# GuildOfWeavers/distaff

Measured on AMD Instinct MI355X. Metric: trace_cells_per_sec, higher is better.
Workload: dtype u128 (prime field 2^128-45*2^40+1, 4x u32 limbs)

## Files before the change

distaff_amd/csrc/air_kernel.h:

```cpp
#pragma once
#include "ctx.h"
#include <type_traits>

#ifndef AIR_THREADS
#define AIR_THREADS 128
#endif
#ifdef AIR_CONVOY
#define AIR_SYNC() __builtin_amdgcn_s_barrier()
#else
#define AIR_SYNC()
#endif
#ifndef AIR_WAVES_PER_SIMD
#define AIR_WAVES_PER_SIMD 2
#endif
constexpr int air_waves_per_simd(int sd, int slcap, int sect) {
    (void)sd; (void)slcap; (void)sect;
#ifdef AIR_WAVES_FORCE
    return AIR_WAVES_FORCE;
#else
    return AIR_WAVES_PER_SIMD;
#endif
}

struct AirConsts { fe sponge_mds[16], sponge_inv_mds[16], hasher_mds[36], hasher_inv_mds[36]; };

struct AirArgs {
    const fe* lde;
    fe* out;
    const fe* coef;
    const fe* tc;
    const fe* periodic;
    const AirConsts* consts;
    fe* partial;
    fe* ev[10];
    const fe* tw_lo; const fe* tw_hi; uint32_t lo_bits;
    unsigned long long* bad_step;
    size_t n, col_stride;
    uint32_t log_n, log_N, log_b, W, ctx_depth, loop_depth, stack_depth;
    uint32_t cl, ll, sl;
    uint32_t coset_step;
    uint32_t q0;
    uint32_t num_inputs, num_outputs;
    fe inputs[8], outputs[8], program_hash[2], op_count;
};



__device__ __forceinline__ fe dpow(const AirArgs& a, uint64_t e) {
    uint32_t l = (uint32_t)e & ((1u << a.lo_bits) - 1u), h = (uint32_t)(e >> a.lo_bits);
    fe v = a.tw_lo[l];
    return h ? fe_mul(v, a.tw_hi[h]) : v;
}

__device__ __forceinline__ fe bnot(const fe& v) { return fe_sub(fe_one(), v); }
__device__ __forceinline__ fe is_bin(const fe& v) { return fe_sub(fe_sqr(v), v); }

template <int Wd>
__device__ __forceinline__ void matmul(fe* s, const fe* m) {
    fe r[Wd];
#pragma unroll
    for (int i = 0; i < Wd; i++) {
        fe_acc A; fe_acc_zero(A);
#pragma unroll
        for (int j = 0; j < Wd; j++) fe_acc_mac(A, m[i * Wd + j], s[j]);
        r[i] = fe_acc_reduce(A);
    }
#pragma unroll
    for (int i = 0; i < Wd; i++) s[i] = r[i];
}

template <int I, int N, class F>
__device__ __forceinline__ void static_for_air(F&& f) {
    if constexpr (I < N) { f(std::integral_constant<int, I>{}); static_for_air<I + 1, N>(f); }
}

struct StackRows { fe o[12], nw[8], hd0; int sl; };
#define ST_AUX0 8
#define ST_AUX1 9

template <int OP, int I> constexpr bool st_has() {
    constexpr bool slot = I < 8, aux0 = I == ST_AUX0, aux1 = I == ST_AUX1;
    switch (OP) {
        case 0x00: case 0x01: case 0x05: case 0x06: case 0x07: return slot || aux0;
        case 0x02: case 0x0E: return slot || aux0;
        case 0x03: case 0x04: case 0x08: case 0x09: case 0x0C: case 0x0D: return slot;
        case 0x0A: case 0x0B: return slot || aux0 || aux1;
        case 0x10: return I >= 1 && slot;
        case 0x11: return I >= 2 && slot;
        case 0x12: case 0x13: case 0x14: case 0x15: return slot;
        case 0x18: return slot && I != 1;
        case 0x19: case 0x1A: case 0x1B: case 0x1C: case 0x1D: return slot;
        default: return false;
    }
}

template <int OP, int I>
__device__ __forceinline__ fe st_term(const StackRows& s) {
    const fe* o = s.o; const fe* nw = s.nw;
    constexpr int i = I < 8 ? I : 0;
    auto L = [&](int num) {
        if (i + num < 8) return fe_sub(o[i + num < 8 ? i + num : 0], nw[i]);
        return i + num < s.sl ? fe_sub(o[i + num < 12 ? i + num : 0], nw[i]) : nw[i];
    };
    auto R = [&](int num) { return fe_sub(o[i - num < 0 ? 0 : i - num], nw[i]); };
    auto C = [&]() { return fe_sub(o[i], nw[i]); };
    auto sel = [&](const fe& c, const fe& x, const fe& y) { return fe_add(y, fe_mul(c, fe_sub(x, y))); };
    if constexpr (OP == 0x00) { if constexpr (I == ST_AUX0) return bnot(o[0]); else return L(1); }
    else if constexpr (OP == 0x01) { if constexpr (I == ST_AUX0) return fe_sub(o[0], o[1]); else return L(2); }
    else if constexpr (OP == 0x02) {
        const fe diff = fe_sub(o[1], o[2]);
        if constexpr (I == ST_AUX0) return fe_mul(nw[0], diff);
        else if constexpr (I == 0) return fe_sub(nw[0], bnot(fe_mul(diff, o[0])));
        else return L(2);
    }
    else if constexpr (OP == 0x03) return L(1);
    else if constexpr (OP == 0x04) return L(4);
    else if constexpr (OP == 0x05) {
        if constexpr (I == ST_AUX0) return is_bin(o[2]);
        else if constexpr (I == 0) return fe_sub(nw[0], sel(o[2], o[0], o[1]));
        else return L(2);
    }
    else if constexpr (OP == 0x06) {
// ... 81 lines not shown
    auto rdiff = [&](int j) { return (SDK != 0 && j >= SDK) ? StDesc{3, 0} : StDesc{2, j}; };
    auto L = [&](int num) { return i + num < 8 ? diff(i + num) : (DEEP ? StDesc{5, -1} : StDesc{3, 0}); };
    auto R = [&](int num) { return diff(i - num < 0 ? 0 : i - num); };
    switch (op) {
        case 0x00: return L(1);
        case 0x01: return L(2);
        case 0x02: return i == 0 ? StDesc{5, -1} : L(2);
        case 0x03: return L(1);
        case 0x04: return L(4);
        case 0x05: return i == 0 ? StDesc{5, -1} : L(2);
        case 0x06: return i < 2 ? (o4_zero ? rdiff(i + 2) : StDesc{5, -1}) : L(4);
        case 0x07: return i < 4 ? (o4_zero ? rdiff(i) : StDesc{5, -1}) : L(2);
        case 0x08: case 0x0B: return i == 0 ? StDesc{5, -1} : L(1);
        case 0x09: case 0x0A: return i == 0 ? StDesc{5, 102} : L(1);
        case 0x0C: case 0x0D: case 0x0E: return i == 0 ? StDesc{5, -1} : diff(i);
        case 0x10: return R(1);
        case 0x11: return R(2);
        case 0x12: return i == 0 ? rdiff(0) : R(1);
        case 0x13: return i < 2 ? rdiff(i) : R(2);
        case 0x14: return i < 4 ? rdiff(i) : R(4);
        case 0x15: return i < 2 ? StDesc{3, 0} : R(2);
        case 0x18: return i == 0 ? StDesc{5, -1} : diff(i);
        case 0x19: return i < 4 ? rdiff(i ^ 2) : diff(i);
        case 0x1A: return rdiff(i ^ 4);
        case 0x1B: return i < 4 ? rdiff((i + 3) & 3) : diff(i);
        case 0x1C: return rdiff((i + 7) & 7);
        case 0x1D: return i == 1 ? StDesc{3, 0} : (i < 4 ? StDesc{5, -1} : diff(i));
        default: return StDesc{0, 0};
    }
}
struct StMerge { int n; int kind[4], j[4], lead[4]; int sgn[4][4]; };
template <int BASE, int I, int SDK, bool DEEP>
constexpr StMerge st_merge() {
    StMerge m{};
    for (int a = 0; a < 4; a++) {
        const StDesc d = st_desc<SDK, DEEP>(BASE + a, I);
        bool has = false;
        switch (a) { case 0: has = st_has<BASE, I>(); break; case 1: has = st_has<BASE + 1, I>(); break; case 2: has = st_has<BASE + 2, I>(); break; default: has = st_has<BASE + 3, I>(); }
        if (!has || d.kind == 0) continue;
        const int cls = d.kind == 5 ? 5 : (d.kind <= 2 ? 1 : 3);
        const int sign = (d.kind == 2 || d.kind == 4) ? -1 : 1;
        int e = -1;
        for (int k = 0; k < m.n; k++) {
            const int kc = m.kind[k] == 5 ? 5 : (m.kind[k] <= 2 ? 1 : 3);
            if (kc != cls) continue;
            if (cls == 3 || (cls == 1 && m.j[k] == d.j) || (cls == 5 && d.j >= 100 && m.j[k] == d.j)) e = k;
        }
        if (e < 0) { e = m.n++; m.kind[e] = d.kind; m.j[e] = d.j; m.lead[e] = a; m.sgn[e][a] = 1; }
        else { const int lead_sign = (m.kind[e] == 2 || m.kind[e] == 4) ? -1 : 1; m.sgn[e][a] = sign * lead_sign; }
    }
    return m;
}

struct StackHigh { fe push, cmp, rescr, keep; fe resc[6]; };

template <int I, uint32_t GROUPS>
__device__ __forceinline__ void st_high_degree(fe_acc& outer, const StackRows& s, const StackHigh& h) {
    if constexpr (I < 8) {
        const fe* o = s.o; const fe* nw = s.nw;
        if constexpr (I >= 1 && (GROUPS & AG_PUSH) != 0) fe_acc_mac(outer, h.push, fe_sub(o[I - 1 < 0 ? 0 : I - 1], nw[I]));
        if constexpr ((GROUPS & AG_CMP) != 0) {
            const fe x_bit = nw[1], y_bit = nw[2], not_set = nw[3];
            fe v;
            if constexpr (I == 0) v = is_bin(x_bit);
            else if constexpr (I == 1) v = is_bin(y_bit);
            else if constexpr (I == 2) v = fe_sub(nw[4], fe_add(o[4], fe_mul(fe_mul(x_bit, bnot(y_bit)), not_set)));
            else if constexpr (I == 3) v = fe_sub(nw[5], fe_add(o[5], fe_mul(fe_mul(y_bit, bnot(x_bit)), not_set)));
            else if constexpr (I == 4) v = fe_sub(nw[6], fe_add(o[6], fe_mul(y_bit, o[0])));
            else if constexpr (I == 5) v = fe_sub(nw[7], fe_add(o[7], fe_mul(x_bit, o[0])));
            else if constexpr (I == 6) v = fe_sub(not_set, fe_mul(bnot(o[5]), bnot(o[4])));
            else v = fe_sub(fe_double(nw[0]), o[0]);
            fe_acc_mac(outer, h.cmp, v);
        }
        if constexpr ((GROUPS & (AG_RESCR | AG_KEEP)) != 0) {
            const fe keep = fe_sub(o[I < 8 ? I : 0], nw[I < 8 ? I : 0]);
            if constexpr ((GROUPS & AG_RESCR) != 0) { if constexpr (I < 6) fe_acc_mac(outer, h.rescr, h.resc[I < 6 ? I : 0]); else fe_acc_mac(outer, h.rescr, keep); }
            if constexpr ((GROUPS & AG_KEEP) != 0) fe_acc_mac(outer, h.keep, keep);
        }
    }
}

template <int I, uint32_t GROUPS> constexpr bool st_touches() {
    if (I >= 8) return (GROUPS & AG_LOW0) != 0;
    return (GROUPS & (AG_LOW0 | AG_LOW1 | AG_HIGH)) != 0;
}

template <int I, uint32_t GROUPS, int SDK, bool DEEP>
__device__ __forceinline__ fe st_output(const StackRows& s, const fe* lo2, const fe& lo0h, const fe* mid, const fe* top, const StackHigh& h) {
    fe_acc outer; fe_acc_zero(outer);
    static_for_air<0, 2>([&](auto c_) {
        constexpr int c = decltype(c_)::value;
        if constexpr (((GROUPS >> (4 * c)) & 0xFu) != 0) {
            fe_acc middle; fe_acc_zero(middle);
            static_for_air<0, 4>([&](auto b_) {
                constexpr int b = decltype(b_)::value;
                constexpr int base = 4 * b + 16 * c;
                if constexpr ((GROUPS & AG_LOW(c, b)) != 0) {
                    static constexpr StMerge M = st_merge<base, I, SDK, DEEP>();
                    if constexpr (M.n > 0) {
                        fe_acc inner; fe_acc_zero(inner);
                        static_for_air<0, M.n>([&](auto e_) {
                            constexpr int e = decltype(e_)::value;
                            fe cf = (base == 0 && M.lead[e] == 0) ? lo0h : lo2[M.lead[e]];
                            static_for_air<0, 4>([&](auto a_) {
                                constexpr int a = decltype(a_)::value;
                                if constexpr (a != M.lead[e] && M.sgn[e][a] != 0) {
                                    const fe other = (base == 0 && a == 0) ? lo0h : lo2[a];
                                    cf = M.sgn[e][a] > 0 ? fe_add(cf, other) : fe_sub(cf, other);
                                }
                            });
                            constexpr int ii = I < 8 ? I : 0;
                            fe term;
                            if constexpr (M.kind[e] == 1) term = fe_sub(s.o[M.j[e]], s.nw[ii]);
                            else if constexpr (M.kind[e] == 2) term = fe_sub(s.nw[ii], s.o[M.j[e]]);
                            else if constexpr (M.kind[e] == 3) term = s.nw[ii];
                            else if constexpr (M.kind[e] == 4) term = fe_neg(s.nw[ii]);
                            else term = st_term<base + M.lead[e], I>(s);
                            fe_acc_mac(inner, cf, term);
                        });
                        fe_acc_mac(middle, mid[b], fe_acc_reduce(inner));
                    }
                }
            });
            fe_acc_mac(outer, top[c], fe_acc_reduce(middle));
        }
    });
    if constexpr ((GROUPS & AG_HIGH) != 0) st_high_degree<I, GROUPS>(outer, s, h);
    return fe_acc_reduce(outer);
}

template <uint32_t ACC_MASK>
struct Acc {
    fe_acc res_acc;
    fe_acc adj_acc[6];
    fe res, adj[6];
    bool nonzero;
    const fe* tc; uint32_t nc;
    __device__ __forceinline__ void emit(uint32_t cidx, int slot, const fe& d) {
        nonzero |= !fe_is_zero(d);
        fe_acc_mac(res_acc, d, tc[cidx]);
        if ((ACC_MASK >> slot) & 1u) fe_acc_mac(adj_acc[slot], d, tc[nc + cidx]);
        else adj[slot] = fe_add(adj[slot], fe_mul(d, tc[nc + cidx]));
    }
};

template <int CL, int LL, int SD, int SLCAP, int SECT, uint32_t GROUPS, int FLAGS>
__global__ void __launch_bounds__(AIR_THREADS, air_waves_per_simd(SD, SLCAP, SECT)) air_kernel(AirArgs a) {
    constexpr bool FIRST = (FLAGS & AF_FIRST) != 0, LAST = (FLAGS & AF_LAST) != 0, EV_IN = (FLAGS & AF_EV_IN) != 0, EV_OUT = (FLAGS & AF_EV_OUT) != 0;
    constexpr int SL = SD ? (SD > 8 ? SD : 8) : SLCAP;
    constexpr bool DEEP = SD == 0 && SLCAP == 12;
    const int cl = (int)a.cl, ll = (int)a.ll;
    const int sl = SD ? SL : (int)a.sl;
    const int sd = SD ? SD : (int)a.stack_depth;
    const fe* c_sponge_mds = a.consts->sponge_mds; const fe* c_sponge_inv_mds = a.consts->sponge_inv_mds;
    const fe* c_hasher_mds = a.consts->hasher_mds; const fe* c_hasher_inv_mds = a.consts->hasher_inv_mds;
    const size_t k = (size_t)blockIdx.x * AIR_THREADS + threadIdx.x;
    if (k >= a.n) return;
    const uint32_t ql = blockIdx.y;
    const uint32_t qg = a.q0 + ql;
    const uint32_t jl = ql * a.coset_step;
    const size_t kn = (k + 1 == a.n) ? 0 : k + 1;
    const fe* cur_p = a.lde + (size_t)jl * a.n + k;
    const fe* nxt_p = a.lde + (size_t)jl * a.n + kn;
    const size_t cs = a.col_stride;
#define CUR(c) cur_p[(size_t)(c) * cs]
#define NXT(c) nxt_p[(size_t)(c) * cs]

    const uint64_t nmask = ((uint64_t)1 << a.log_N) - 1;
    const uint64_t gi = ((uint64_t)k << a.log_b) + (uint64_t)qg * a.coset_step;
    const uint32_t step = (uint32_t)(((uint64_t)k << 3) + qg);
    const uint64_t n64 = a.n;

    const fe c_opc = CUR(0), n_opc = NXT(0);
    fe c_sp[4], n_sp[4], cf[3], ld[5], hd[2], n_cf[3];
#pragma unroll
    for (int i = 0; i < 4; i++) { c_sp[i] = CUR(1 + i); n_sp[i] = NXT(1 + i); }
#pragma unroll
    for (int i = 0; i < 3; i++) { cf[i] = CUR(5 + i); n_cf[i] = NXT(5 + i); }
#pragma unroll
    for (int i = 0; i < 5; i++) ld[i] = CUR(8 + i);
#pragma unroll
    for (int i = 0; i < 2; i++) hd[i] = CUR(13 + i);
    fe c_ctx[CL], n_ctx[CL], c_lp[LL], n_lp[LL], o[SL], nw[SL];
    {
        uint32_t col = 15;
#pragma unroll
        for (int i = 0; i < CL; i++) { bool on = (uint32_t)i < a.ctx_depth; c_ctx[i] = on ? CUR(col + i) : fe_zero(); n_ctx[i] = on ? NXT(col + i) : fe_zero(); }
        col += a.ctx_depth;
#pragma unroll
        for (int i = 0; i < LL; i++) { bool on = (uint32_t)i < a.loop_depth; c_lp[i] = on ? CUR(col + i) : fe_zero(); n_lp[i] = on ? NXT(col + i) : fe_zero(); }
        col += a.loop_depth;
#pragma unroll
        for (int i = 0; i < SL; i++) { bool on = i < sd; o[i] = on ? CUR(col + i) : fe_zero(); nw[i] = on ? NXT(col + i) : fe_zero(); }
    }

    if constexpr ((SECT & 1) != 0) {
        const fe xp = dpow(a, (gi * (6 * n64 + 2)) & nmask);
        const fe one = fe_one();
#pragma unroll 1
        for (int pass = 0; pass < 2; pass++) {
            const fe* cc = a.coef + pass * 94;
            fe_acc R, A; fe_acc_zero(R); fe_acc_zero(A);
            auto term = [&](const fe& v, uint32_t idx) { fe_acc_mac(R, v, cc[idx]); fe_acc_mac(A, v, cc[idx + 1]); };
            term(pass ? fe_sub(c_opc, a.op_count) : c_opc, 0);
            if (pass == 0) { for (int i = 0; i < 4; i++) term(c_sp[i], 2 + 2 * i); }
            else { for (int i = 0; i < 2; i++) term(fe_sub(c_sp[i], a.program_hash[i]), 2 + 2 * i); }
            for (int i = 0; i < 3; i++) term(pass ? fe_sub(cf[i], one) : cf[i], 10 + 2 * i);
            for (int i = 0; i < 5; i++) term(pass ? fe_sub(ld[i], one) : ld[i], 16 + 2 * i);
            for (int i = 0; i < 2; i++) term(pass ? fe_sub(hd[i], one) : hd[i], 26 + 2 * i);
            for (int i = 0; i < CL; i++) if (i < cl) term(c_ctx[i], 30 + 2 * i);
            for (int i = 0; i < LL; i++) if (i < ll) term(c_lp[i], 62 + 2 * i);
            const uint32_t nio = pass ? a.num_outputs : a.num_inputs;
// ... 121 lines not shown
                fe_acc_mac(A, ccpy, fe_sub(c_ctx[i], n_ctx[i]));
                const fe v = fe_acc_reduce(A);
                acc.emit(20 + i, 2, v);
            }
#pragma unroll
            for (int i = 0; i < LL; i++) {
                if (i >= ll) break;
                fe v = fe_mul(lcpy, fe_sub(c_lp[i], n_lp[i]));
                if (i >= 1) v = fe_add(v, fe_mul(f_loop, fe_sub(c_lp[i - 1 < 0 ? 0 : i - 1], n_lp[i])));
                v = fe_add(v, fe_mul(f_break, i + 1 < ll ? fe_sub(c_lp[i + 1 < LL ? i + 1 : 0], n_lp[i]) : n_lp[i]));
                acc.emit(20 + cl + i, 2, v);
            }
        } else {
            auto ctx_cur = [&](int i) { return (uint32_t)i < a.ctx_depth ? CUR(15 + i) : fe_zero(); };
            auto ctx_nxt = [&](int i) { return (uint32_t)i < a.ctx_depth ? NXT(15 + i) : fe_zero(); };
            const uint32_t lcol = 15 + a.ctx_depth;
            auto lp_cur = [&](int i) { return (uint32_t)i < a.loop_depth ? CUR(lcol + i) : fe_zero(); };
            auto lp_nxt = [&](int i) { return (uint32_t)i < a.loop_depth ? NXT(lcol + i) : fe_zero(); };
#pragma unroll 1
            for (int i = 0; i < cl; i++) {
                const fe ni = ctx_nxt(i);
                fe_acc A; fe_acc_zero(A);
                fe_acc_mac(A, push, fe_sub(i == 0 ? c_sp[0] : ctx_cur(i - 1), ni));
                fe_acc_mac(A, pop, i + 1 < cl ? fe_sub(ctx_cur(i + 1), ni) : ni);
                fe_acc_mac(A, ccpy, fe_sub(ctx_cur(i), ni));
                acc.emit(20 + i, 2, fe_acc_reduce(A));
            }
#pragma unroll 1
            for (int i = 0; i < ll; i++) {
                const fe ni = lp_nxt(i);
                fe_acc A; fe_acc_zero(A);
                fe_acc_mac(A, lcpy, fe_sub(lp_cur(i), ni));
                if (i >= 1) fe_acc_mac(A, f_loop, fe_sub(lp_cur(i - 1), ni));
                fe_acc_mac(A, f_break, i + 1 < ll ? fe_sub(lp_cur(i + 1), ni) : ni);
                acc.emit(20 + cl + i, 2, fe_acc_reduce(A));
            }
        }
    }

    constexpr bool NESTED = SD == 4 || (SD == 0 && SLCAP == 8) || DEEP;
    static_assert(NESTED ? (SECT & 120) == 0 : GROUPS == 0, "nested-sum instances select stack operations with GROUPS, the per-operation instance with SECT");
    if constexpr (NESTED && (GROUPS & AG_STACK_ALL & ~AG_DEEP) != 0) {
        constexpr int NS = SD == 4 ? 4 : 8;
        StackRows rows;
#pragma unroll
        for (int i = 0; i < 8; i++) { rows.o[i] = o[i]; rows.nw[i] = nw[i]; }
#pragma unroll
        for (int i = 8; i < 12; i++) rows.o[i] = DEEP ? o[i < SL ? i : 0] : fe_zero();
        rows.hd0 = hd[0];
        rows.sl = DEEP ? sl : 8;
        const fe lo0h = fe_mul(lo2[0], hd[0]);
        StackHigh high;
        high.push = hdf[0]; high.cmp = hdf[1]; high.rescr = hdf[2]; high.keep = fe_add(begin_flag, noop_flag);
        if constexpr ((GROUPS & AG_RESCR) != 0) {
            constexpr int NZ = (SD != 0 && SD < 6) ? SD : 6;
            fe os[6], ns[6];
#pragma unroll
            for (int i = 0; i < 6; i++) os[i] = i < NZ ? fe_cube(fe_add(o[i], per[8 + i])) : per[23 + i];
            matmul<6>(os, c_hasher_mds);
            constexpr int NR = NS < 6 ? NS : 6;
#pragma unroll
            for (int i = 0; i < NR; i++) {
                fe_acc A; fe_acc_zero(A);
#pragma unroll
                for (int j = 0; j < NZ; j++) fe_acc_mac(A, c_hasher_inv_mds[i * 6 + j], nw[j]);
                ns[i] = fe_acc_reduce(A);
            }
#pragma unroll
            for (int i = 0; i < NR; i++) high.resc[i] = fe_sub(fe_sub(fe_cube(ns[i]), per[14 + i]), os[i]);
        }
        AIR_SYNC();
        const uint32_t sbase = 20 + cl + ll;
        static_for_air<0, NS + 2>([&](auto k_) {
            constexpr int kk = decltype(k_)::value;
            constexpr int I = kk < NS ? kk : (kk == NS ? ST_AUX0 : ST_AUX1);
            constexpr bool touched = st_touches<I, GROUPS>();
            if constexpr (touched || !EV_OUT) {
                if (I >= 8 || I < sd) {
                    fe v = fe_zero();
                    if constexpr (touched) v = st_output<I, GROUPS, SD, DEEP>(rows, lo2, lo0h, mid, top, high);
                    fe* slot = a.ev[I] + pidx;
                    if constexpr (EV_IN) v = touched ? fe_add(v, *slot) : *slot;
                    if constexpr (EV_OUT) *slot = v;
                    else acc.emit(I >= 8 ? sbase + (I - 8) : sbase + 2 + I, 4, v);
                }
            } else if constexpr (!EV_IN) {
                a.ev[I][pidx] = fe_zero();
            }
            AIR_SYNC();
        });
    }
    if constexpr (!NESTED && (SECT & 120) != 0) {
        constexpr int SLR = SL;
        fe ev[SLR], aux0 = fe_zero(), aux1 = fe_zero();
#pragma unroll
        for (int i = 0; i < SLR; i++) ev[i] = fe_zero();
        auto agg = [&](int i, const fe& f, const fe& v) { if (i < sd) ev[i] = fe_add(ev[i], fe_mul(f, v)); };
        auto copy_from = [&](int from, const fe& f) {
#pragma unroll
            for (int i = 0; i < SLR; i++) if (i >= from && i < sl) agg(i, f, fe_sub(o[i], nw[i]));
        };
        auto rshift = [&](int num, const fe& f) {
#pragma unroll
            for (int i = 0; i < SLR; i++) if (i >= num && i < sl) agg(i, f, fe_sub(o[i - num < 0 ? 0 : i - num], nw[i]));
        };
        auto lshift = [&](int from, int num, const fe& f) {
#pragma unroll
            for (int i = 0; i < SLR; i++) {
                if (i >= from - num && i < sl - num) agg(i, f, fe_sub(o[i + num < SL ? i + num : 0], nw[i]));
                else if (i >= sl - num && i < sl) agg(i, f, nw[i]);
            }
        };
        fe f;
        constexpr bool HD_FUSED = false;
        if constexpr (!NESTED && (SECT & 8) != 0) {
        f = LDF(0x12); agg(0, f, fe_sub(nw[0], o[0]));
        rshift(1, fe_add(LDF(0x10), f));
        f = LDF(0x13); agg(0, f, fe_sub(nw[0], o[0])); agg(1, f, fe_sub(nw[1], o[1]));
        f = LDF(0x15); agg(0, f, nw[0]); agg(1, f, nw[1]);
        rshift(2, fe_add(fe_add(LDF(0x11), LDF(0x13)), LDF(0x15)));
        f = LDF(0x14);
#pragma unroll
        for (int i = 0; i < 4; i++) agg(i, f, fe_sub(nw[i], o[i]));
        rshift(4, f);
        lshift(1, 1, fe_add(assert_flag, LDF(0x03)));
        aux0 = fe_add(aux0, fe_mul(assert_flag, fe_sub(fe_one(), o[0])));
        lshift(2, 2, LDF(0x01));
        aux0 = fe_add(aux0, fe_mul(LDF(0x01), fe_sub(o[0], o[1])));
        lshift(4, 4, LDF(0x04));
        f = LDF(0x18); agg(0, f, fe_sub(nw[0], o[1])); agg(0, f, fe_sub(nw[1], o[0])); copy_from(2, f);
        f = LDF(0x19); agg(0, f, fe_sub(nw[0], o[2])); agg(1, f, fe_sub(nw[1], o[3])); agg(2, f, fe_sub(nw[2], o[0])); agg(3, f, fe_sub(nw[3], o[1])); copy_from(4, f);
        f = LDF(0x1A);
#pragma unroll
// ... 66 lines not shown
            f = hdf[1];
            fe x_bit = nw[1], y_bit = nw[2], not_set = nw[3];
            agg(0, f, is_bin(x_bit)); agg(1, f, is_bin(y_bit));
            fe bit_gt = fe_mul(x_bit, bnot(y_bit)), bit_lt = fe_mul(y_bit, bnot(x_bit));
            agg(2, f, fe_sub(nw[4], fe_add(o[4], fe_mul(bit_gt, not_set))));
            agg(3, f, fe_sub(nw[5], fe_add(o[5], fe_mul(bit_lt, not_set))));
            agg(4, f, fe_sub(nw[6], fe_add(o[6], fe_mul(y_bit, o[0]))));
            agg(5, f, fe_sub(nw[7], fe_add(o[7], fe_mul(x_bit, o[0]))));
            agg(6, f, fe_sub(not_set, fe_mul(bnot(o[5]), bnot(o[4]))));
            agg(7, f, fe_sub(fe_double(nw[0]), o[0]));
            copy_from(8, f);
        }
        copy_from(0, fe_add(begin_flag, noop_flag));
        }
        if constexpr (!HD_FUSED && (SECT & 64) != 0) {
        {
            f = hdf[2];
            fe os[6], ns[6];
#pragma unroll
            for (int i = 0; i < 6; i++) os[i] = fe_cube(fe_add(o[i], per[8 + i]));
            matmul<6>(os, c_hasher_mds);
#pragma unroll
            for (int i = 0; i < 6; i++) ns[i] = nw[i];
            matmul<6>(ns, c_hasher_inv_mds);
#pragma unroll
            for (int i = 0; i < 6; i++) ns[i] = fe_sub(fe_cube(ns[i]), per[14 + i]);
#pragma unroll
            for (int i = 0; i < 6; i++) agg(i, f, fe_sub(ns[i], os[i]));
            copy_from(6, f);
        }
        }

        const uint32_t sbase = 20 + cl + ll;
        if constexpr ((SECT & 40) != 0) { acc.emit(sbase, 4, aux0); acc.emit(sbase + 1, 4, aux1); }
#pragma unroll
        for (int i = 0; i < SLR; i++) if (i < sd) acc.emit(sbase + 2 + i, 4, ev[i]);
    }
    if constexpr (DEEP && (GROUPS & AG_DEEP) != 0) {
        {
            const uint32_t sbase = 20 + cl + ll;
            const fe lo_all = fe_add(fe_add(lo2[0], lo2[1]), fe_add(lo2[2], lo2[3]));
            fe fl1, fl2, fl4, fr1, fr2, fr4, fcp;
            { fe_acc A; fe_acc_zero(A); fe_acc_mac(A, mid[0], lo2[3]); fe_acc_mac(A, mid[2], lo_all); fl1 = fe_add(fe_mul(top[0], fe_acc_reduce(A)), assert_flag); }
            { fe_acc A; fe_acc_zero(A); fe_acc_mac(A, mid[0], fe_add(lo2[1], lo2[2])); fe_acc_mac(A, mid[1], fe_add(lo2[1], lo2[3])); fl2 = fe_mul(top[0], fe_acc_reduce(A)); }
            fl4 = fe_mul(top[0], fe_mul(mid[1], fe_add(lo2[0], lo2[2])));
            fr1 = fe_add(fe_mul(top[1], fe_mul(mid[0], fe_add(lo2[0], lo2[2]))), hdf[0]);
            { fe_acc A; fe_acc_zero(A); fe_acc_mac(A, mid[0], fe_add(lo2[1], lo2[3])); fe_acc_mac(A, mid[1], lo2[1]); fr2 = fe_mul(top[1], fe_acc_reduce(A)); }
            fr4 = fe_mul(top[1], fe_mul(mid[1], lo2[0]));
            {
                fe_acc A; fe_acc_zero(A); fe_acc_mac(A, mid[2], lo_all); fe_acc_mac(A, mid[3], fe_add(lo2[0], lo2[1]));
                fe_acc B; fe_acc_zero(B); fe_acc_mac(B, top[1], fe_acc_reduce(A)); fe_acc_mac(B, top[0], fe_mul(mid[3], fe_add(fe_add(lo2[0], lo2[1]), lo2[2])));
                fcp = fe_add(fe_add(fe_acc_reduce(B), fe_add(hdf[1], hdf[2])), fe_add(begin_flag, noop_flag));
            }
            const uint32_t scol = 15 + a.ctx_depth + a.loop_depth;
#pragma unroll 1
            for (int i = 8; i < sd; i++) {
                const fe ni = NXT(scol + i);
                auto item = [&](int j) { return CUR(scol + j); };
                auto left = [&](int num) { return i + num < sl ? fe_sub(item(i + num), ni) : ni; };
                fe_acc A; fe_acc_zero(A);
                fe_acc_mac(A, fcp, fe_sub(item(i), ni));
                fe_acc_mac(A, fr1, fe_sub(item(i - 1), ni)); fe_acc_mac(A, fr2, fe_sub(item(i - 2), ni)); fe_acc_mac(A, fr4, fe_sub(item(i - 4), ni));
                fe_acc_mac(A, fl1, left(1)); fe_acc_mac(A, fl2, left(2)); fe_acc_mac(A, fl4, left(4));
                acc.emit(sbase + 2 + i, 4, fe_acc_reduce(A));
            }
        }
    }

    if constexpr (SECT == 1) return;
    const bool on_trace = (qg == 0);
    if (on_trace && k + 1 != a.n && acc.nonzero) atomicMin(a.bad_step, (unsigned long long)k);
    acc.res = fe_acc_reduce(acc.res_acc);
    constexpr bool EMITS_STACK = (SECT & 120) != 0 || (GROUPS & AG_DEEP) != 0 || ((GROUPS & AG_STACK_ALL) != 0 && !EV_OUT);
    constexpr uint32_t USED = ((SECT & 2) ? 0x2Fu : 0u) | ((SECT & 4) ? 0x18u : 0u) | ((SECT & 128) ? 0x04u : 0u) | (EMITS_STACK ? 0x10u : 0u);
#pragma unroll
    for (int i = 0; i < 6; i++) if (((ACC_MASK & USED) >> i) & 1u) acc.adj[i] = fe_add(acc.adj[i], fe_acc_reduce(acc.adj_acc[i]));
    if constexpr (!FIRST) {
        acc.res = fe_add(acc.res, a.partial[pidx]);
#pragma unroll
        for (int i = 0; i < 6; i++) if (LAST || ((USED >> i) & 1u)) acc.adj[i] = fe_add(acc.adj[i], a.partial[(size_t)(i + 1) * pstride + pidx]);
    }
    if constexpr (!LAST) {
        a.partial[pidx] = acc.res;
#pragma unroll
        for (int i = 0; i < 6; i++) if (FIRST || ((USED >> i) & 1u)) a.partial[(size_t)(i + 1) * pstride + pidx] = acc.adj[i];
        return;
    }
    fe t;
    if (on_trace && k + 1 != a.n) {
        t = fe_zero();
    } else {
        const uint32_t degs[6] = {2, 3, 4, 6, 7, 8};
        fe_acc T; fe_acc_zero(T);
        fe_acc_add(T, acc.res);
#pragma unroll
        for (int g = 0; g < 6; g++) {
            uint64_t p = 8 * n64 - 1 - (n64 - 1) * degs[g];
            fe_acc_mac(T, acc.adj[g], dpow(a, (gi * p) & nmask));
        }
        t = fe_acc_reduce(T);
    }
    a.out[((size_t)2 * gridDim.y + ql) * a.n + k] = t;
#undef CUR
#undef NXT
}


template <int CL, int LL, int SD, int SLCAP, int SECT, uint32_t GROUPS, int FLAGS>
static void launch_air(dst_ctx* c, const AirArgs& a, uint32_t Q) {
    dim3 g((unsigned)((c->n + AIR_THREADS - 1) / AIR_THREADS), Q);
    static char name[64];
    if (!name[0]) snprintf(name, sizeof(name), "air_kernel<%d,%d,%d,%d,%d,%u,%d>", CL, LL, SD, SLCAP, SECT, (unsigned)GROUPS, FLAGS);
    constexpr int NS = SD == 4 ? 6 : 10;
    const double units = c->W + ((FLAGS & AF_FIRST) ? 0 : 7) + ((FLAGS & AF_LAST) ? 1 : 7) + ((SECT & 1) ? 2 : 0) + ((FLAGS & AF_EV_IN) ? NS : 0) + ((FLAGS & AF_EV_OUT) ? NS : 0);
    { KScope ks_(c, name, 16.0 * c->n * Q * units, true); hipLaunchKernelGGL((air_kernel<CL, LL, SD, SLCAP, SECT, GROUPS, FLAGS>), g, dim3(AIR_THREADS), 0, c->stream, a); }
}
void air_launch_sd4(dst_ctx* c, const AirArgs& a, uint32_t Q);
void air_launch_small(dst_ctx* c, const AirArgs& a, uint32_t Q);
void air_launch_deep(dst_ctx* c, const AirArgs& a, uint32_t Q);
void air_launch_generic(dst_ctx* c, const AirArgs& a, uint32_t Q);
```

distaff_amd/csrc/ctx.h:

```cpp
#pragma once
#include <hip/hip_runtime.h>
#include <stdint.h>
#include <string.h>
#include <memory>
#include <string>
#include <map>
#include <vector>
#include "fe.h"
#include "../../include/distaff_hip.h"

struct __attribute__((aligned(16))) digest { uint32_t w[8]; };
#define AIR_PERIODIC_STRIDE 29

#ifndef NTT_TW4_PAIRS
#define NTT_TW4_PAIRS 0
#endif
#if NTT_TW4_PAIRS
typedef fe_tw tw4_t;
#else
typedef fe tw4_t;
#endif

#define DST_MAX_FRI_LAYERS 24

struct dst_switch_def { const char* name; bool product; const char* values; const char* what; };
static const dst_switch_def DST_SWITCHES[] = {
    {"DISTAFF_SHARD_DEBUG",        true,  "1",               "stderr line per tree exchange on rank 0; communicators record the order of their collectives (dst_comm_trace)"},
    {"DISTAFF_SHARD_TREE_GATHER",  true,  "1",               "sharded Merkle trees: all-gather of all boundary nodes + upper levels repeated on every rank (BASELINE north_star's all-gather-only form) instead of the k-range all-to-all"},
    {"DISTAFF_SHARD_NO_OVERLAP",   true,  "1",               "sharded prover: every collective on the context's main stream (no second stream / events) also on a stream-ordered transport"},
    {"DISTAFF_COMM_TIMEOUT_S",     true,  "seconds",         "communicators: limit of every host wait behind a collective (default 60; <= 0: none); on expiry the rank aborts the communicator and returns DST_ERR_COMM (dst_comm_set_timeout changes it per handle)"},
    {"DISTAFF_LOCAL_TRANSPORT",    true,  "blocking",        "in-process transport (dst_comm_init_local, dst_prove_sharded_local): drain every rank's stream around each collective instead of the stream-ordered form (events between the ranks' streams, nothing waited for)"},
    {"DISTAFF_TMP_REGS",           true,  "4..W",            "registers per transform launch = size of the staging array (default: as many as 12 GiB hold, at most W)"},
    {"DISTAFF_AIR",                false, "small|deep|generic", "force a more general constraint-kernel instance set than the trace shape needs (generic = per-operation formulation)"},
    {"DISTAFF_BOUNDARY",           false, "eval",            "boundary combinations by evaluation on the 8n domain (the reference's route) instead of coefficient form"},
    {"DISTAFF_COMBINE",            false, "steps",           "combine_polys / DEEP composition as the reference's sequence of whole-array steps instead of the fused passes"},
    {"DISTAFF_NTT",                false, "pre|3pass|reg|lds", "force a transform plan family"},
    {"DISTAFF_NTT_SHAPE",          false, "a,b",             "three-pass plans: log2 of the first two pass lengths"},
    {"DISTAFF_NTT_ORDER",          false, "0",               "first pass of an extension in coset-slow block order"},
    {"DISTAFF_NTT_WAVES",          false, "4|8",             "force the 512- or 1024-lane instances of the LDS passes"},
    {"DISTAFF_NTT_FIXED",          false, "0",               "use the any-shape instances where a shape-compiled one exists"},
    {"DISTAFF_NTT_DIF",            false, "0|1|2",           "first pass of an extension: coset DIT (0), pre-scale + DIF (1), DIT with last-stage twiddles from global memory (2)"},
    {"DISTAFF_NTT_DEBUG",          false, "1",               "print the occupancy of every transform launch shape once"},
    {"DISTAFF_LDE_BATCH",          false, "cols,cosets",     "registers x cosets per transform launch"},
    {"DISTAFF_FOLD8_DFT",          false, "0",               "8n-coefficient extensions without the fused fold + 8-point step"},
    {"DISTAFF_TRACE_BUFFER",       false, "1",               "give the trace its own buffer instead of coset 0 of the extension"},
    {"DISTAFF_MERKLE_LEVEL2_LOG",  false, "k",               "build two tree levels per launch from 2^k nodes on (default 2^15)"},
    {"DISTAFF_MERKLE_LEVELS",      false, "1",               "one launch per tree level"},
    {"DISTAFF_SYN_DIV_TABLES",     false, "1",               "synthetic division by power tables + scan instead of the blocked form"},
    {"DISTAFF_FRI_TAIL",           false, "0",               "no single-launch tail: every FRI layer by its own launches (the tail otherwise starts at the first layer of at most 2^13 elements)"},
    {"DISTAFF_FRI_CHAIN",          false, "0",               "FRI commit phase with a root read-back and a host draw per layer"},
    {"DISTAFF_FRI_REPLICATE_LOG",  false, "k",               "sharded prover: replicate FRI layers from 2^k elements on (default 2^17)"},
    {"DISTAFF_SHARD_FORCE_OVERLAP", false, "1",              "sharded prover: the two-stream choreography of a stream-ordered transport over a blocking one"},
    {"DISTAFF_TEST_STALL_COLLECTIVE", false, "k|k@r",        "communicators: fault injection -- before device collective number k (of rank r only) a kernel holds the stream until the communicator is aborted"},
};
enum : size_t {
    HS_WEIGHTS = 0,
    HS_WEIGHTS_BYTES = (4 * 128 + 4) * 16,
    HS_DEEP = 32768,
    HS_DEEP_HALF = 2048,
    HS_FRI_ROOTS = 40960,
    HS_FRI_SLOTS = 45056,
    HS_FRI_SLOT_BYTES = 800,
    HS_AIR_FLAG = 65536 - 64,
    HS_DRAWS = 65536,
    HS_DRAWS_BYTES = (344 + 160) * 16,
    HS_COMPOSE = 65536 + 8192,
    HS_COMPOSE_BYTES = 516 * 16,
    HS_STATUS = 65536 + 8192 + 8320,
    HS_STATUS_SLOTS = 32,
    HS_TREE_READBACK = 65536 + 8192 + 8320 + 2048,
    HS_TAIL_ROOTS = HS_TREE_READBACK + 1024,
    HS_POW = HS_TAIL_ROOTS + 1024,
    HS_TOTAL = 131072
};
static_assert(HS_WEIGHTS + HS_WEIGHTS_BYTES <= HS_DEEP, "boundary weights overlap the DEEP values");
static_assert(HS_DEEP_HALF >= 128 * 16 && HS_DEEP + 2 * HS_DEEP_HALF <= HS_FRI_ROOTS, "DEEP values: W <= 128 registers");
static_assert(HS_FRI_ROOTS + DST_MAX_FRI_LAYERS * 32 <= HS_FRI_SLOTS, "FRI roots overlap the layer slots");
static_assert(8 * 96 + 32 <= HS_FRI_SLOT_BYTES && HS_FRI_SLOTS + DST_MAX_FRI_LAYERS * HS_FRI_SLOT_BYTES <= HS_AIR_FLAG, "FRI layer slots: G <= 8 ranks, DST_MAX_FRI_LAYERS layers");
static_assert(HS_DRAWS + HS_DRAWS_BYTES <= HS_COMPOSE && HS_COMPOSE + HS_COMPOSE_BYTES <= HS_STATUS && HS_STATUS + HS_STATUS_SLOTS * 64 <= HS_TOTAL, "upload regions overlap");
static_assert(HS_STATUS_SLOTS >= 2 + DST_MAX_FRI_LAYERS, "one status slot per tree exchange of a proof");
static_assert(HS_STATUS + HS_STATUS_SLOTS * 64 <= HS_TREE_READBACK && 8 * 96 + 32 <= 1024 && DST_MAX_FRI_LAYERS * 32 <= 1024 && HS_POW + 64 <= HS_TOTAL, "read-back regions overlap");

#ifdef DISTAFF_TEST_HOOKS
#define DST_TEST_HOOKS 1
#else
#define DST_TEST_HOOKS 0
// ... 232 lines not shown
```

distaff_amd/csrc/kernels_air.hip:

```cpp
#include "air_kernel.h"
#include "rescue_constants.h"

#if DST_TEST_HOOKS
void air_launch_generic(dst_ctx* c, const AirArgs& a, uint32_t Q) {
    launch_air<16, 8, 0, 32, 2, 0, AF_FIRST>(c, a, Q);
    if (dst_internal_boundary_by_evaluation(c)) launch_air<16, 8, 0, 32, 1, 0, 0>(c, a, Q);
    launch_air<16, 8, 0, 32, 132, 0, 0>(c, a, Q);
    launch_air<16, 8, 0, 32, 8, 0, 0>(c, a, Q);
    launch_air<16, 8, 0, 32, 32, 0, 0>(c, a, Q);
    launch_air<16, 8, 0, 32, 16, 0, 0>(c, a, Q);
    launch_air<16, 8, 0, 32, 64, 0, AF_LAST>(c, a, Q);
}
#endif


int k_constraint_check(dst_ctx* c, int64_t* bad_step) {
    const unsigned long long res = c->air_flag_host;
    if (res != ~0ull) { if (bad_step) *bad_step = (int64_t)res; return DST_ERR_AIR; }
    if (bad_step) *bad_step = -1;
    return DST_OK;
}
int k_eval_constraints(dst_ctx* c, const fe* coeffs_dev, const fe* tc_dev, int64_t* bad_step, bool defer_check) {
    if (!c->air_consts) {
        AirConsts h;
        memcpy(h.sponge_mds, SPONGE_MDS, sizeof(h.sponge_mds)); memcpy(h.sponge_inv_mds, SPONGE_INV_MDS, sizeof(h.sponge_inv_mds));
        memcpy(h.hasher_mds, HASHER_MDS, sizeof(h.hasher_mds)); memcpy(h.hasher_inv_mds, HASHER_INV_MDS, sizeof(h.hasher_inv_mds));
        HIP_TRY(c, hipMalloc(&c->air_consts, sizeof(AirConsts)));
        HIP_TRY(c, hipMemcpy(c->air_consts, &h, sizeof(AirConsts), hipMemcpyHostToDevice));
    }
    AirArgs a{};
    a.lde = c->lde; a.out = c->ceval; a.coef = coeffs_dev; a.tc = tc_dev; a.periodic = c->periodic; a.consts = (const AirConsts*)c->air_consts; a.partial = c->cwork;
    {
        const size_t per = (size_t)(c->Bc / (c->B / 8)) * c->n;
        if (8 * per > c->Bc * c->tmp_regs * c->n) { c->err = "constraint evaluation: staging buffer too small for the stack partial values"; return DST_ERR_STATE; }
        for (int i = 0; i < 8; i++) a.ev[i] = c->tmp + (size_t)i * per;
        a.ev[8] = c->cpoly; a.ev[9] = c->comp_poly;
    }
    a.tw_lo = c->tw_lo; a.tw_hi = c->tw_hi; a.lo_bits = c->tw_lo_bits;
    a.bad_step = (unsigned long long*)c->d_u64;
    a.n = c->n; a.col_stride = c->Bc * c->n;
    a.log_n = c->log_n; a.log_N = c->log_N; a.log_b = c->log_b; a.W = (uint32_t)c->W;
    a.ctx_depth = c->prm.ctx_depth; a.loop_depth = c->prm.loop_depth; a.stack_depth = (uint32_t)c->stack_depth;
    a.coset_step = (uint32_t)(c->B / 8);
    a.q0 = (uint32_t)(c->j0 / (c->B / 8));
    uint32_t Q = (uint32_t)(c->Bc / (c->B / 8));
    a.num_inputs = c->pub.num_inputs; a.num_outputs = c->pub.num_outputs;
    memcpy(a.inputs, c->pub.inputs, sizeof(a.inputs)); memcpy(a.outputs, c->pub.outputs, sizeof(a.outputs));
    memcpy(a.program_hash, c->program_hash, sizeof(a.program_hash));
    a.op_count = fe_from_u64(c->op_count);
    HIP_TRY(c, hipMemsetAsync(c->d_u64, 0xFF, 8, c->stream));
    const uint32_t cd = c->prm.ctx_depth, lp = c->prm.loop_depth, sd = (uint32_t)c->stack_depth;
    a.cl = cd > 1 ? cd : 1; a.ll = lp > 1 ? lp : 1; a.sl = sd > 8 ? sd : 8;
    const char* force = c->sw("DISTAFF_AIR");
    const bool want_generic = force && !strcmp(force, "generic"), want_small = force && !strcmp(force, "small"), want_deep = force && !strcmp(force, "deep");
    const bool general = want_generic || want_deep;
    if (a.cl <= 2 && a.ll <= 1 && sd == 4 && !general && !want_small) air_launch_sd4(c, a, Q);
    else if (a.cl <= 2 && a.ll <= 1 && sd <= 8 && !general) air_launch_small(c, a, Q);
#if DST_TEST_HOOKS
    else if (want_generic) air_launch_generic(c, a, Q);
#endif
    else air_launch_deep(c, a, Q);
    unsigned long long* flag = c->h_stage ? reinterpret_cast<unsigned long long*>(c->h_stage + HS_AIR_FLAG) : &c->air_flag_host;
    HIP_TRY(c, hipMemcpyAsync(flag, c->d_u64, 8, hipMemcpyDeviceToHost, c->stream));
    if (defer_check && c->h_stage) return DST_OK;
    HIP_TRY(c, hipStreamSynchronize(c->stream));
    c->air_flag_host = *flag;
    return k_constraint_check(c, bad_step);
}
```

Measured before the change: 595.3 million.

## Skip constraint groups whose flag is zero across a wavefront on trace coset

New measurement: 594.8 million. Within noise of the previous version (-0.1%).

```diff
diff --git a/distaff_amd/csrc/air_kernel.h b/distaff_amd/csrc/air_kernel.h
--- a/distaff_amd/csrc/air_kernel.h
+++ b/distaff_amd/csrc/air_kernel.h
@@ -41,6 +41,7 @@
     uint32_t coset_step;
     uint32_t q0;
     uint32_t num_inputs, num_outputs;
+    uint32_t sparse;
     fe inputs[8], outputs[8], program_hash[2], op_count;
 };
 
@@ -68,6 +69,35 @@
 #pragma unroll
     for (int i = 0; i < Wd; i++) s[i] = r[i];
 }
+
+struct AirWave {
+    bool on;
+#if defined(DISTAFF_EMULATED)
+    uint32_t phase;
+#endif
+};
+__device__ __forceinline__ bool air_wave_zero(AirWave& w, const fe& v) {
+#if defined(DISTAFF_EMULATED)
+    static __shared__ unsigned char votes[2][AIR_THREADS];
+    unsigned char* slot = votes[w.phase++ & 1u];
+    slot[threadIdx.x] = fe_is_zero(v) ? 0 : 1;
+    __syncthreads();
+    const unsigned lane0 = threadIdx.x & ~63u;
+    unsigned any = 0;
+    for (unsigned i = 0; i < 64 && lane0 + i < AIR_THREADS; i++) any |= slot[lane0 + i];
+    return any == 0;
+#else
+    return __ballot(!fe_is_zero(v)) == 0ull;
+#endif
+}
+#define SK_LO(a) (1u << (a))
+#define SK_LO0H 0x10u
+#define SK_MID(b) (0x20u << (b))
+#define SK_TOP(c) (0x200u << (c))
+#define SK_PUSH 0x800u
+#define SK_CMP 0x1000u
+#define SK_RESCR 0x2000u
+#define SK_KEEP 0x4000u
 
 template <int I, int N, class F>
 __device__ __forceinline__ void static_for_air(F&& f) {
@@ -255,14 +285,25 @@
     return m;
 }
 
+template <int SDK, bool DEEP, uint32_t GROUPS> constexpr int st_guard_level() {
+    if (SDK != 0) return 3;
+    if (DEEP && (GROUPS & AG_LOW0) == (AG_LOW(0, 1) | AG_LOW(0, 3))) return 0;
+    return 2;
+}
+constexpr uint32_t st_members(const StMerge& m, int e, int base) {
+    uint32_t r = 0;
+    for (int a = 0; a < 4; a++) if (a == m.lead[e] || m.sgn[e][a] != 0) r |= (base == 0 && a == 0) ? SK_LO0H : SK_LO(a);
+    return r;
+}
+
 struct StackHigh { fe push, cmp, rescr, keep; fe resc[6]; };
 
 template <int I, uint32_t GROUPS>
-__device__ __forceinline__ void st_high_degree(fe_acc& outer, const StackRows& s, const StackHigh& h) {
+__device__ __forceinline__ void st_high_degree(fe_acc& outer, const StackRows& s, const StackHigh& h, uint32_t skip) {
     if constexpr (I < 8) {
         const fe* o = s.o; const fe* nw = s.nw;
-        if constexpr (I >= 1 && (GROUPS & AG_PUSH) != 0) fe_acc_mac(outer, h.push, fe_sub(o[I - 1 < 0 ? 0 : I - 1], nw[I]));
-        if constexpr ((GROUPS & AG_CMP) != 0) {
+        if constexpr (I >= 1 && (GROUPS & AG_PUSH) != 0) { if (!(skip & SK_PUSH)) fe_acc_mac(outer, h.push, fe_sub(o[I - 1 < 0 ? 0 : I - 1], nw[I])); }
+        if constexpr ((GROUPS & AG_CMP) != 0) if (!(skip & SK_CMP)) {
             const fe x_bit = nw[1], y_bit = nw[2], not_set = nw[3];
             fe v;
             if constexpr (I == 0) v = is_bin(x_bit);
@@ -276,9 +317,12 @@
             fe_acc_mac(outer, h.cmp, v);
         }
         if constexpr ((GROUPS & (AG_RESCR | AG_KEEP)) != 0) {
-            const fe keep = fe_sub(o[I < 8 ? I : 0], nw[I < 8 ? I : 0]);
-            if constexpr ((GROUPS & AG_RESCR) != 0) { if constexpr (I < 6) fe_acc_mac(outer, h.rescr, h.resc[I < 6 ? I : 0]); else fe_acc_mac(outer, h.rescr, keep); }
-            if constexpr ((GROUPS & AG_KEEP) != 0) fe_acc_mac(outer, h.keep, keep);
+            constexpr uint32_t both = ((GROUPS & AG_RESCR) ? SK_RESCR : 0u) | ((GROUPS & AG_KEEP) ? SK_KEEP : 0u);
+            if ((~skip & both) != 0) {
+                const fe keep = fe_sub(o[I < 8 ? I : 0], nw[I < 8 ? I : 0]);
+                if constexpr ((GROUPS & AG_RESCR) != 0) if (!(skip & SK_RESCR)) { if constexpr (I < 6) fe_acc_mac(outer, h.rescr, h.resc[I < 6 ? I : 0]); else fe_acc_mac(outer, h.rescr, keep); }
+                if constexpr ((GROUPS & AG_KEEP) != 0) if (!(skip & SK_KEEP)) fe_acc_mac(outer, h.keep, keep);
+            }
         }
     }
 }
@@ -289,21 +333,26 @@
 }
 
 template <int I, uint32_t GROUPS, int SDK, bool DEEP>
-__device__ __forceinline__ fe st_output(const StackRows& s, const fe* lo2, const fe& lo0h, const fe* mid, const fe* top, const StackHigh& h) {
+__device__ __forceinline__ fe st_output(const StackRows& s, const fe* lo2, const fe& lo0h, const fe* mid, const fe* top, const StackHigh& h, uint32_t skip = 0) {
+    constexpr int LEVEL = st_guard_level<SDK, DEEP, GROUPS>();
     fe_acc outer; fe_acc_zero(outer);
     static_for_air<0, 2>([&](auto c_) {
         constexpr int c = decltype(c_)::value;
-        if constexpr (((GROUPS >> (4 * c)) & 0xFu) != 0) {
+        if constexpr (((GROUPS >> (4 * c)) & 0xFu) != 0) if (!(skip & SK_TOP(c))) {
             fe_acc middle; fe_acc_zero(middle);
             static_for_air<0, 4>([&](auto b_) {
                 constexpr int b = decltype(b_)::value;
                 constexpr int base = 4 * b + 16 * c;
                 if constexpr ((GROUPS & AG_LOW(c, b)) != 0) {
                     static constexpr StMerge M = st_merge<base, I, SDK, DEEP>();
-                    if constexpr (M.n > 0) {
+                    if constexpr (M.n > 0) if (!(LEVEL >= 2 && (skip & SK_MID(b)))) {
                         fe_acc inner; fe_acc_zero(inner);
                         static_for_air<0, M.n>([&](auto e_) {
                             constexpr int e = decltype(e_)::value;
+                            if constexpr (LEVEL >= 3) {
+                                constexpr uint32_t members = st_members(M, e, base);
+                                if ((~skip & members) == 0) return;
+                            }
                             fe cf = (base == 0 && M.lead[e] == 0) ? lo0h : lo2[M.lead[e]];
                             static_for_air<0, 4>([&](auto a_) {
                                 constexpr int a = decltype(a_)::value;
@@ -328,7 +377,7 @@
             fe_acc_mac(outer, top[c], fe_acc_reduce(middle));
         }
     });
-    if constexpr ((GROUPS & AG_HIGH) != 0) st_high_degree<I, GROUPS>(outer, s, h);
+    if constexpr ((GROUPS & AG_HIGH) != 0) st_high_degree<I, GROUPS>(outer, s, h, skip);
     return fe_acc_reduce(outer);
 }
 
@@ -361,6 +410,9 @@
     if (k >= a.n) return;
     const uint32_t ql = blockIdx.y;
     const uint32_t qg = a.q0 + ql;
+    const bool on_trace = (qg == 0);
+    AirWave wave{};
+    wave.on = on_trace && a.sparse != 0;
     const uint32_t jl = ql * a.coset_step;
     const size_t kn = (k + 1 == a.n) ? 0 : k + 1;
     const fe* cur_p = a.lde + (size_t)jl * a.n + k;
@@ -588,7 +640,26 @@
         const fe lo0h = fe_mul(lo2[0], hd[0]);
         StackHigh high;
         high.push = hdf[0]; high.cmp = hdf[1]; high.rescr = hdf[2]; high.keep = fe_add(begin_flag, noop_flag);
-        if constexpr ((GROUPS & AG_RESCR) != 0) {
+        uint32_t skip = 0;
+        if (wave.on) {
+            constexpr int LEVEL = st_guard_level<SD, DEEP, GROUPS>();
+            if constexpr ((GROUPS & (AG_LOW0 | AG_LOW1)) != 0 && LEVEL >= 3) {
+#pragma unroll
+                for (int i = 0; i < 4; i++) if (air_wave_zero(wave, lo2[i])) skip |= SK_LO(i);
+            }
+            if constexpr ((GROUPS & (AG_LOW0 | AG_LOW1)) != 0 && LEVEL >= 2) {
+#pragma unroll
+                for (int b = 0; b < 4; b++) if (((GROUPS | (GROUPS >> 4)) >> b) & 1u) { if (air_wave_zero(wave, mid[b])) skip |= SK_MID(b); }
+            }
+            if constexpr ((GROUPS & AG_LOW0) != 0 && LEVEL >= 1) { if (air_wave_zero(wave, top[0])) skip |= SK_TOP(0); }
+            if constexpr ((GROUPS & AG_LOW(0, 0)) != 0 && LEVEL >= 3) { if (air_wave_zero(wave, lo0h)) skip |= SK_LO0H; }
+            if constexpr ((GROUPS & AG_LOW1) != 0 && LEVEL >= 1) { if (air_wave_zero(wave, top[1])) skip |= SK_TOP(1); }
+            if constexpr ((GROUPS & AG_PUSH) != 0) { if (air_wave_zero(wave, high.push)) skip |= SK_PUSH; }
+            if constexpr ((GROUPS & AG_CMP) != 0) { if (air_wave_zero(wave, high.cmp)) skip |= SK_CMP; }
+            if constexpr ((GROUPS & AG_RESCR) != 0) { if (air_wave_zero(wave, high.rescr)) skip |= SK_RESCR; }
+            if constexpr ((GROUPS & AG_KEEP) != 0) { if (air_wave_zero(wave, high.keep)) skip |= SK_KEEP; }
+        }
+        if constexpr ((GROUPS & AG_RESCR) != 0) if (!(skip & SK_RESCR)) {
             constexpr int NZ = (SD != 0 && SD < 6) ? SD : 6;
             fe os[6], ns[6];
 #pragma unroll
@@ -614,7 +685,7 @@
             if constexpr (touched || !EV_OUT) {
                 if (I >= 8 || I < sd) {
                     fe v = fe_zero();
-                    if constexpr (touched) v = st_output<I, GROUPS, SD, DEEP>(rows, lo2, lo0h, mid, top, high);
+                    if constexpr (touched) v = st_output<I, GROUPS, SD, DEEP>(rows, lo2, lo0h, mid, top, high, skip);
                     fe* slot = a.ev[I] + pidx;
                     if constexpr (EV_IN) v = touched ? fe_add(v, *slot) : *slot;
                     if constexpr (EV_OUT) *slot = v;
@@ -787,6 +858,12 @@
                 fe_acc B; fe_acc_zero(B); fe_acc_mac(B, top[1], fe_acc_reduce(A)); fe_acc_mac(B, top[0], fe_mul(mid[3], fe_add(fe_add(lo2[0], lo2[1]), lo2[2])));
                 fcp = fe_add(fe_add(fe_acc_reduce(B), fe_add(hdf[1], hdf[2])), fe_add(begin_flag, noop_flag));
             }
+            uint32_t skip = 0;
+            if (wave.on) {
+                const fe* sums[7] = {&fcp, &fr1, &fr2, &fr4, &fl1, &fl2, &fl4};
+#pragma unroll
+                for (int j = 0; j < 7; j++) if (air_wave_zero(wave, *sums[j])) skip |= 1u << j;
+            }
             const uint32_t scol = 15 + a.ctx_depth + a.loop_depth;
 #pragma unroll 1
             for (int i = 8; i < sd; i++) {
@@ -794,16 +871,19 @@
                 auto item = [&](int j) { return CUR(scol + j); };
                 auto left = [&](int num) { return i + num < sl ? fe_sub(item(i + num), ni) : ni; };
                 fe_acc A; fe_acc_zero(A);
-                fe_acc_mac(A, fcp, fe_sub(item(i), ni));
-                fe_acc_mac(A, fr1, fe_sub(item(i - 1), ni)); fe_acc_mac(A, fr2, fe_sub(item(i - 2), ni)); fe_acc_mac(A, fr4, fe_sub(item(i - 4), ni));
-                fe_acc_mac(A, fl1, left(1)); fe_acc_mac(A, fl2, left(2)); fe_acc_mac(A, fl4, left(4));
+                if (!(skip & 1u)) fe_acc_mac(A, fcp, fe_sub(item(i), ni));
+                if (!(skip & 2u)) fe_acc_mac(A, fr1, fe_sub(item(i - 1), ni));
+                if (!(skip & 4u)) fe_acc_mac(A, fr2, fe_sub(item(i - 2), ni));
+                if (!(skip & 8u)) fe_acc_mac(A, fr4, fe_sub(item(i - 4), ni));
+                if (!(skip & 16u)) fe_acc_mac(A, fl1, left(1));
+                if (!(skip & 32u)) fe_acc_mac(A, fl2, left(2));
+                if (!(skip & 64u)) fe_acc_mac(A, fl4, left(4));
                 acc.emit(sbase + 2 + i, 4, fe_acc_reduce(A));
             }
         }
     }
 
     if constexpr (SECT == 1) return;
-    const bool on_trace = (qg == 0);
     if (on_trace && k + 1 != a.n && acc.nonzero) atomicMin(a.bad_step, (unsigned long long)k);
     acc.res = fe_acc_reduce(acc.res_acc);
     constexpr bool EMITS_STACK = (SECT & 120) != 0 || (GROUPS & AG_DEEP) != 0 || ((GROUPS & AG_STACK_ALL) != 0 && !EV_OUT);
diff --git a/distaff_amd/csrc/ctx.h b/distaff_amd/csrc/ctx.h
--- a/distaff_amd/csrc/ctx.h
+++ b/distaff_amd/csrc/ctx.h
@@ -32,6 +32,7 @@
     {"DISTAFF_LOCAL_TRANSPORT",    true,  "blocking",        "in-process transport (dst_comm_init_local, dst_prove_sharded_local): drain every rank's stream around each collective instead of the stream-ordered form (events between the ranks' streams, nothing waited for)"},
     {"DISTAFF_TMP_REGS",           true,  "4..W",            "registers per transform launch = size of the staging array (default: as many as 12 GiB hold, at most W)"},
     {"DISTAFF_AIR",                false, "small|deep|generic", "force a more general constraint-kernel instance set than the trace shape needs (generic = per-operation formulation)"},
+    {"DISTAFF_AIR_SPARSE",         false, "0",               "constraint kernels: no skipping of operation groups whose flag is zero in a whole wavefront on the trace coset (the dense form everywhere)"},
     {"DISTAFF_BOUNDARY",           false, "eval",            "boundary combinations by evaluation on the 8n domain (the reference's route) instead of coefficient form"},
     {"DISTAFF_COMBINE",            false, "steps",           "combine_polys / DEEP composition as the reference's sequence of whole-array steps instead of the fused passes"},
     {"DISTAFF_NTT",                false, "pre|3pass|reg|lds", "force a transform plan family"},
diff --git a/distaff_amd/csrc/kernels_air.hip b/distaff_amd/csrc/kernels_air.hip
--- a/distaff_amd/csrc/kernels_air.hip
+++ b/distaff_amd/csrc/kernels_air.hip
@@ -51,6 +51,7 @@
     HIP_TRY(c, hipMemsetAsync(c->d_u64, 0xFF, 8, c->stream));
     const uint32_t cd = c->prm.ctx_depth, lp = c->prm.loop_depth, sd = (uint32_t)c->stack_depth;
     a.cl = cd > 1 ? cd : 1; a.ll = lp > 1 ? lp : 1; a.sl = sd > 8 ? sd : 8;
+    a.sparse = c->sw_is("DISTAFF_AIR_SPARSE", "0") ? 0u : 1u;
     const char* force = c->sw("DISTAFF_AIR");
     const bool want_generic = force && !strcmp(force, "generic"), want_small = force && !strcmp(force, "small"), want_deep = force && !strcmp(force, "deep");
     const bool general = want_generic || want_deep;
```
